# adrianalbert/domain-transfer-GAN

Hardware: AMD Instinct MI355X
Metric: training images/sec, 256x256 Augmented CycleGAN step, 1/2/4/8 MI355X (higher is better)
Workload: dtype f32 tensors; conv products as 3 bf16 MFMAs on hi/lo-split fp32 operands (~2^-17 operand rounding), fp32 accumulate; parity vs the reference goldens: losses / single-pass images / cycle reconstructions <= 1e-3 on every fixture at step 0 (measured rec_A / rec_B <= 7.9e-4, profiles/r06_rec_errors.txt)

## Files before the change

### domain-transfer-gan_amd/csrc/conv_patch.hip

```cpp
#include "common.h"
#include "conv_internal.h"

typedef __bf16 bf16x8 __attribute__((ext_vector_type(8)));
typedef float f32x4 __attribute__((ext_vector_type(4)));
typedef unsigned u32x4 __attribute__((ext_vector_type(4)));

namespace {
constexpr int PT_TH = 8, PT_TW = 16;
constexpr int PT_PIX = 320;
constexpr int PT_PLANE = PT_PIX * 8;
constexpr int PT_IMG = 4 * PT_PLANE;
}

template <bool REFLECT>
__global__ __launch_bounds__(256) void conv_patch16_x3(const float *__restrict__ in, const __bf16 *__restrict__ wp,
                                                       const float *__restrict__ bias, float *__restrict__ out, Geom g,
                                                       Taps taps, int dymin, int dxmin, int PH, int PW, unsigned in_bytes,
                                                       long long w_lo_elems)
{
    __shared__ __attribute__((aligned(16))) __bf16 Ap[2 * PT_IMG];
    const int tid = threadIdx.x, lane = tid & 63, wave = __builtin_amdgcn_readfirstlane(tid >> 6);
    const int tiles_x = (g.GW + PT_TW - 1) / PT_TW, tiles_y = (g.GH + PT_TH - 1) / PT_TH;
    const int nwg_ = gridDim.x, bid_ = blockIdx.x, xq_ = nwg_ >> 3, xr_ = nwg_ & 7, xcd_ = bid_ & 7;
    int b = (xcd_ < xr_ ? xcd_ * (xq_ + 1) : xr_ * (xq_ + 1) + (xcd_ - xr_) * xq_) + (bid_ >> 3);
    const int tx = b % tiles_x; b /= tiles_x;
    const int ty = b % tiles_y;
    const int n = b / tiles_y;
    const int gy0 = ty * PT_TH, gx0 = tx * PT_TW;

    const __amdgpu_buffer_rsrc_t rin = __builtin_amdgcn_make_buffer_rsrc((void *)in, 0, in_bytes, 0x00020000);
    const int npp = PH * PW;
    constexpr int NIT = 4 * PT_PIX / 256;
    static_assert(4 * PT_PIX % 256 == 0, "patch items per thread");
    f32x4 plo[NIT], phi[NIT];
#pragma unroll
    for (int it = 0; it < NIT; ++it) {
        const int i = tid + 256 * it;
        const int u = i / PT_PIX, pp = i - u * PT_PIX;
        const int py = pp / PW, px = pp - py * PW;
        int iy = gy0 + py + dymin, ix = gx0 + px + dxmin;
        bool ok = pp < npp;
        if (REFLECT) {
            ok = ok && iy > -g.Hin && iy < 2 * g.Hin - 1 && ix > -g.Win && ix < 2 * g.Win - 1;
            iy = iy < 0 ? -iy : iy;
            iy = iy >= g.Hin ? 2 * (g.Hin - 1) - iy : iy;
            ix = ix < 0 ? -ix : ix;
            ix = ix >= g.Win ? 2 * (g.Win - 1) - ix : ix;
        } else {
            ok = ok && (unsigned)iy < (unsigned)g.Hin && (unsigned)ix < (unsigned)g.Win;
        }
        const unsigned off = (unsigned)(((n * g.Hin + iy) * g.Win + ix) * g.Cin + 8 * u) * 4u;
        plo[it] = __builtin_bit_cast(f32x4, __builtin_amdgcn_raw_buffer_load_b128(rin, acg_masked_off(off, ok), 0, 0));
        phi[it] = __builtin_bit_cast(f32x4, __builtin_amdgcn_raw_buffer_load_b128(rin, acg_masked_off(off + 16u, ok), 0, 0));
    }
#pragma unroll
    for (int it = 0; it < NIT; ++it) {
        const int i = tid + 256 * it;
        const int u = i / PT_PIX, pp = i - u * PT_PIX;
        if (pp >= npp) continue;
        const float v[8] = {plo[it][0], plo[it][1], plo[it][2], plo[it][3], phi[it][0], phi[it][1], phi[it][2], phi[it][3]};
        acg_u32x4 hi, lo;
        acg_split8(v, hi, lo);
        *(acg_u32x4 *)&Ap[u * PT_PLANE + pp * 8] = hi;
        *(acg_u32x4 *)&Ap[PT_IMG + u * PT_PLANE + pp * 8] = lo;
    }
    __syncthreads();

    const int pl = lane >> 4, lr = lane & 15;
    f32x4 acc[2] = {{0.f, 0.f, 0.f, 0.f}, {0.f, 0.f, 0.f, 0.f}};
    const long long boff = ((long long)(pl >> 1) * g.ncols_pad + lr) * 16 + (pl & 1) * 8;
    const long long tap_stride = (long long)(g.Cin / 16) * g.ncols_pad * 16;
    constexpr int PF = 7;
    const int tap_v = taps.pk[lane < taps.n ? lane : 0];
    bf16x8 bh[PF], bl[PF];
    auto bload = [&](int t, bf16x8 &h, bf16x8 &l) {
        const int tw = __builtin_amdgcn_readlane(tap_v, t < taps.n ? t : 0) >> 16;
        const __bf16 *wt = wp + tw * tap_stride + boff;
        h = *(const bf16x8 *)wt;
        l = *(const bf16x8 *)(wt + w_lo_elems);
    };
    auto tap_mma = [&](int t, const bf16x8 &ch, const bf16x8 &cl) {
        const int pk = __builtin_amdgcn_readlane(tap_v, t);
        const int dy = ((pk << 24) >> 24) - dymin, dx = ((pk << 16) >> 24) - dxmin;
#pragma unroll
        for (int r = 0; r < 2; ++r) {
            const int pp = (wave * 2 + r + dy) * PW + dx + lr;
            const bf16x8 ah = *(const bf16x8 *)&Ap[pl * PT_PLANE + pp * 8];
            const bf16x8 al = *(const bf16x8 *)&Ap[PT_IMG + pl * PT_PLANE + pp * 8];
            acc[r] = __builtin_amdgcn_mfma_f32_16x16x32_bf16(al, ch, acc[r], 0, 0, 0);
            acc[r] = __builtin_amdgcn_mfma_f32_16x16x32_bf16(ah, cl, acc[r], 0, 0, 0);
            acc[r] = __builtin_amdgcn_mfma_f32_16x16x32_bf16(ah, ch, acc[r], 0, 0, 0);
        }
    };
    const int nfull = taps.n / PF * PF;
    if (nfull > 0) {
#pragma unroll
        for (int j = 0; j < PF; ++j) bload(j, bh[j], bl[j]);
    }
    for (int t0 = 0; t0 < nfull; t0 += PF) {
#pragma unroll
        for (int j = 0; j < PF; ++j) {
            tap_mma(t0 + j, bh[j], bl[j]);
            bload(t0 + j + PF, bh[j], bl[j]);
        }
    }
    for (int t = nfull; t < taps.n; ++t) {
        bf16x8 ch, cl;
        bload(t, ch, cl);
        tap_mma(t, ch, cl);
    }

    const float bv = (bias != nullptr && lr < g.Cout) ? bias[lr] : 0.f;
#pragma unroll
    for (int r = 0; r < 2; ++r) {
        const int gy = gy0 + wave * 2 + r;
#pragma unroll
        for (int k = 0; k < 4; ++k) {
            const int gx = gx0 + 4 * pl + k;
            if (gy < g.GH && gx < g.GW && lr < g.Cout)
                out[(((long long)n * g.Hout + gy) * g.Wout + gx) * g.Cout + lr] = acg_apply_act_ch(acc[r][k] + bv, g.act, lr);
        }
    }
}

template <bool REFLECT>
__global__ __launch_bounds__(256) __attribute__((amdgpu_waves_per_eu(4, 4))) void conv_patchn_x3(const float *__restrict__ in, const __bf16 *__restrict__ wn,
                                                      const float *__restrict__ bias, float *__restrict__ out, Geom g,
                                                      int dymin, int dxmin, int KH, int KW, unsigned in_bytes)
{
    __shared__ __attribute__((aligned(16))) __bf16 Ap[2 * PT_IMG];
    const int tid = threadIdx.x, lane = tid & 63, wave = __builtin_amdgcn_readfirstlane(tid >> 6);
    const int tiles_x = (g.GW + PT_TW - 1) / PT_TW, tiles_y = (g.GH + PT_TH - 1) / PT_TH;
    const int nwg_ = gridDim.x, bid_ = blockIdx.x, xq_ = nwg_ >> 3, xr_ = nwg_ & 7, xcd_ = bid_ & 7;
    int b = (xcd_ < xr_ ? xcd_ * (xq_ + 1) : xr_ * (xq_ + 1) + (xcd_ - xr_) * xq_) + (bid_ >> 3);
    const int tx = b % tiles_x; b /= tiles_x;
    const int ty = b % tiles_y;
    const int n = b / tiles_y;
    const int gy0 = ty * PT_TH, gx0 = tx * PT_TW;
    const int PH = PT_TH + KH - 1, PW = PT_TW + KW - 1;

    const __amdgpu_buffer_rsrc_t rin = __builtin_amdgcn_make_buffer_rsrc((void *)in, 0, in_bytes, 0x00020000);
    const int npp = PH * PW;
    constexpr int NIT = 4 * PT_PIX / 256;
    f32x4 plo[NIT], phi[NIT];
#pragma unroll
    for (int it = 0; it < NIT; ++it) {
        const int i = tid + 256 * it;
        const int u = i / PT_PIX, pp = i - u * PT_PIX;
        const int py = pp / PW, px = pp - py * PW;
        int iy = gy0 + py + dymin, ix = gx0 + px + dxmin;
        bool ok = pp < npp;
        if (REFLECT) {
            ok = ok && iy > -g.Hin && iy < 2 * g.Hin - 1 && ix > -g.Win && ix < 2 * g.Win - 1;
            iy = iy < 0 ? -iy : iy;
            iy = iy >= g.Hin ? 2 * (g.Hin - 1) - iy : iy;
            ix = ix < 0 ? -ix : ix;
            ix = ix >= g.Win ? 2 * (g.Win - 1) - ix : ix;
        } else {
            ok = ok && (unsigned)iy < (unsigned)g.Hin && (unsigned)ix < (unsigned)g.Win;
        }
        const unsigned off = (unsigned)(((n * g.Hin + iy) * g.Win + ix) * g.Cin + 8 * u) * 4u;
        plo[it] = __builtin_bit_cast(f32x4, __builtin_amdgcn_raw_buffer_load_b128(rin, acg_masked_off(off, ok), 0, 0));
        phi[it] = __builtin_bit_cast(f32x4, __builtin_amdgcn_raw_buffer_load_b128(rin, acg_masked_off(off + 16u, ok), 0, 0));
    }
    const int KU = KW + 3, S = KH * KU;
    constexpr int NSW = (7 * 10 + 3) / 4, PF = 6;
    bf16x8 bh[PF], bl[PF];
    auto bload = [&](int k, bf16x8 &h, bf16x8 &l) {
        int s = wave + 4 * k;
        s = s < S ? s : S - 1;
        h = *(const bf16x8 *)(wn + (long long)s * 512 + lane * 8);
        l = *(const bf16x8 *)(wn + (long long)(S + s) * 512 + lane * 8);
    };
#pragma unroll
    for (int k = 0; k < PF; ++k) bload(k, bh[k], bl[k]);
#pragma unroll
    for (int it = 0; it < NIT; ++it) {
        const int i = tid + 256 * it;
        const int u = i / PT_PIX, pp = i - u * PT_PIX;
        if (pp >= npp) continue;
        const float v[8] = {plo[it][0], plo[it][1], plo[it][2], plo[it][3], phi[it][0], phi[it][1], phi[it][2], phi[it][3]};
        acg_u32x4 hi, lo;
        acg_split8(v, hi, lo);
        *(acg_u32x4 *)&Ap[u * PT_PLANE + pp * 8] = hi;
        *(acg_u32x4 *)&Ap[PT_IMG + u * PT_PLANE + pp * 8] = lo;
    }
    __syncthreads();

    const int kg = lane >> 4, m = lane & 15, br = m >> 2, bc = m & 3;
    f32x4 acc[2] = {{0.f, 0.f, 0.f, 0.f}, {0.f, 0.f, 0.f, 0.f}};
    const int a0 = kg * PT_PLANE + (br * PW + 4 * bc) * 8;
#pragma unroll
    for (int k = 0; k < NSW; ++k) {
        const int s = wave + 4 * k;
        if (s < S) {
            const int ry = s / KU, u = s - ry * KU;
#pragma unroll
            for (int mt = 0; mt < 2; ++mt) {
                const int e = a0 + ((4 * mt + ry) * PW + u) * 8;
                const bf16x8 ah = *(const bf16x8 *)&Ap[e];
                const bf16x8 al = *(const bf16x8 *)&Ap[PT_IMG + e];
                acc[mt] = __builtin_amdgcn_mfma_f32_16x16x32_bf16(al, bh[k % PF], acc[mt], 0, 0, 0);
                acc[mt] = __builtin_amdgcn_mfma_f32_16x16x32_bf16(ah, bl[k % PF], acc[mt], 0, 0, 0);
                acc[mt] = __builtin_amdgcn_mfma_f32_16x16x32_bf16(ah, bh[k % PF], acc[mt], 0, 0, 0);
            }
        }
        if (k + PF < NSW) bload(k + PF, bh[k % PF], bl[k % PF]);
    }
    __syncthreads();
    float *red = (float *)Ap;
#pragma unroll
    for (int mt = 0; mt < 2; ++mt)
#pragma unroll
        for (int r = 0; r < 4; ++r) red[((wave * 2 + mt) * 4 + r) * 64 + lane] = acc[mt][r];
    __syncthreads();
    if (wave < 2) {
        const int mt = wave, c = lane & 3, dxo = (lane >> 2) & 3, q = lane >> 4;
        const float bv = (bias != nullptr && c < g.Cout) ? bias[c] : 0.f;
        const int gy = gy0 + 4 * mt + q;
#pragma unroll
        for (int r = 0; r < 4; ++r) {
            float v = red[((0 * 2 + mt) * 4 + r) * 64 + lane];
#pragma unroll
            for (int w = 1; w < 4; ++w) v += red[((w * 2 + mt) * 4 + r) * 64 + lane];
            const int gx = gx0 + 4 * r + dxo;
            if (gy < g.GH && gx < g.GW)
                out[(((long long)n * g.Hout + gy) * g.Wout + gx) * 4 + c] = acg_apply_act_ch(v + bv, g.act, c);
        }
    }
}

static bool patchn_window(const Taps &t, int *ymin, int *xmin, int *KH, int *KW)
{
    int y0 = t.dy[0], y1 = t.dy[0], x0 = t.dx[0], x1 = t.dx[0];
    for (int i = 1; i < t.n; ++i) {
        y0 = t.dy[i] < y0 ? t.dy[i] : y0; y1 = t.dy[i] > y1 ? t.dy[i] : y1;
        x0 = t.dx[i] < x0 ? t.dx[i] : x0; x1 = t.dx[i] > x1 ? t.dx[i] : x1;
    }
    const int kh = y1 - y0 + 1, kw = x1 - x0 + 1;
    if (kh != kw || kh * kw != t.n || kh < 2 || kh > 7) return false;
    unsigned long long seen = 0;
    bool all_fwd = true, all_bwd = true;
    for (int i = 0; i < t.n; ++i) {
        const int pos = (t.dy[i] - y0) * kw + (t.dx[i] - x0);
        if (seen >> pos & 1ull) return false;
        seen |= 1ull << pos;
        const int skh = t.w[i] / kw, skw = t.w[i] - skh * kw;
        all_fwd = all_fwd && skh == t.dy[i] - y0 && skw == t.dx[i] - x0;
        all_bwd = all_bwd && skh == kh - 1 - (t.dy[i] - y0) && skw == kw - 1 - (t.dx[i] - x0);
    }
    if (!all_fwd && !all_bwd) return false;
    *ymin = y0; *xmin = x0; *KH = kh; *KW = kw;
    return true;
}

bool acg_conv_patchn_ok(const Geom &g, const Taps &t)
{
    if (g_acg_precision != ACG_PREC_BF16X3 || g_acg_conv_impl != ACG_IMPL_MFMA || g.thin || g.fold_p || g.stats) return false;
    if (g.Cin != 32 || g.Cout != 4 || g.os != 1 || g.is != 1 || g.oy0 != 0 || g.ox0 != 0 || t.n < 4) return false;
    int a, b, kh, kw;
    if (!patchn_window(t, &a, &b, &kh, &kw)) return false;
    return (PT_TH + kh - 1) * (PT_TW + kw - 1) <= PT_PIX && g.Hin >= 2 && g.Win >= 2;
}

int acg_conv_patchn_launch(const float *in, const void *wn, const float *bias, float *out, const Geom &g, const Taps &t, hipStream_t st)
{
    int ymin, xmin, KH, KW;
    ACG_REQUIRE(acg_conv_patchn_ok(g, t) && patchn_window(t, &ymin, &xmin, &KH, &KW), "conv_patchn_x3: unsupported geometry");
    const long long nimg = g.Mtot / ((long long)g.GH * g.GW);
    const long long in_bytes = nimg * g.Hin * g.Win * g.Cin * 4;
    ACG_REQUIRE(in_bytes < (1LL << 32), "conv_patchn_x3: gathered tensor exceeds the 4 GiB buffer-addressing limit");
    const long long blocks = nimg * ((g.GH + PT_TH - 1) / PT_TH) * ((g.GW + PT_TW - 1) / PT_TW);
    if (g.reflect)
        hipLaunchKernelGGL((conv_patchn_x3<true>), dim3((unsigned)blocks), dim3(256), 0, st, in, (const __bf16 *)wn, bias, out, g, ymin, xmin, KH, KW, (unsigned)in_bytes);
    else
        hipLaunchKernelGGL((conv_patchn_x3<false>), dim3((unsigned)blocks), dim3(256), 0, st, in, (const __bf16 *)wn, bias, out, g, ymin, xmin, KH, KW, (unsigned)in_bytes);
    ACG_CHECK_LAUNCH("conv_patchn_x3");
    acg_note_kernel("conv_patchn_x3<REFLECT=%d> (%dx%d window, %d K steps)", g.reflect ? 1 : 0, KH, KW, KH * (KW + 3));
    return ACG_OK;
}

namespace {
constexpr int TR_PW = PT_TW + 8;
constexpr int TR_PHMAX = PT_TH + 6;
constexpr int TR_PLANE = TR_PHMAX * TR_PW * 4;
}
template <bool REFLECT>
__global__ __launch_bounds__(256) void conv_thinrow_x3(const float *__restrict__ in, const __bf16 *__restrict__ wr,
                                                       const float *__restrict__ bias, float *__restrict__ out, Geom g,
                                                       int dymin, int dxmin, int KH, unsigned in_bytes)
{
    __shared__ __attribute__((aligned(16))) float smem[PT_TH * PT_TW * 32 + 512];
    static_assert(sizeof(smem) >= 2 * TR_PLANE * sizeof(__bf16), "patch fits the tile buffer");
    __bf16 *const Ap = (__bf16 *)smem;
    const int tid = threadIdx.x, lane = tid & 63, wave = __builtin_amdgcn_readfirstlane(tid >> 6);
    const int tiles_x = (g.GW + PT_TW - 1) / PT_TW, tiles_y = (g.GH + PT_TH - 1) / PT_TH;
    const int nwg_ = gridDim.x, bid_ = blockIdx.x, xq_ = nwg_ >> 3, xr_ = nwg_ & 7, xcd_ = bid_ & 7;
    int b = (xcd_ < xr_ ? xcd_ * (xq_ + 1) : xr_ * (xq_ + 1) + (xcd_ - xr_) * xq_) + (bid_ >> 3);
    const int tx = b % tiles_x; b /= tiles_x;
    const int ty = b % tiles_y;
    const int n = b / tiles_y;
    const int gy0 = ty * PT_TH, gx0 = tx * PT_TW;
    const int PH = PT_TH + KH - 1;

    constexpr int PF = 3;
    const int kg = lane >> 4, lr = lane & 15;
    bf16x8 bh[PF][2], bl[PF][2];
    auto bload = [&](int ry, bf16x8 (&h)[2], bf16x8 (&l)[2]) {
        const int r = ry < KH ? ry : KH - 1;
#pragma unroll
        for (int ct = 0; ct < 2; ++ct) {
            const long long e = ((long long)(r * 4 + kg) * 32 + ct * 16 + lr) * 8;
            h[ct] = *(const bf16x8 *)(wr + e);
            l[ct] = *(const bf16x8 *)(wr + (long long)KH * 1024 + e);
        }
    };
#pragma unroll
    for (int k = 0; k < PF; ++k) bload(k, bh[k], bl[k]);

    const __amdgpu_buffer_rsrc_t rin = __builtin_amdgcn_make_buffer_rsrc((void *)in, 0, in_bytes, 0x00020000);
    constexpr int NIT = (TR_PHMAX * TR_PW + 255) / 256;
    f32x4 pv[NIT];
#pragma unroll
    for (int it = 0; it < NIT; ++it) {
        const int pp = tid + 256 * it;
        const int py = pp / TR_PW, px = pp - py * TR_PW;
        int iy = gy0 + py + dymin, ix = gx0 + px + dxmin;
        bool ok = py < PH;
        if (REFLECT) {
            ok = ok && iy > -g.Hin && iy < 2 * g.Hin - 1 && ix > -g.Win && ix < 2 * g.Win - 1;
            iy = iy < 0 ? -iy : iy;
            iy = iy >= g.Hin ? 2 * (g.Hin - 1) - iy : iy;
            ix = ix < 0 ? -ix : ix;
            ix = ix >= g.Win ? 2 * (g.Win - 1) - ix : ix;
        } else {
            ok = ok && (unsigned)iy < (unsigned)g.Hin && (unsigned)ix < (unsigned)g.Win;
        }
        const unsigned off = (unsigned)(((n * g.Hin + iy) * g.Win + ix) * 4) * 4u;
        pv[it] = __builtin_bit_cast(f32x4, __builtin_amdgcn_raw_buffer_load_b128(rin, acg_masked_off(off, ok), 0, 0));
    }
#pragma unroll
    for (int it = 0; it < NIT; ++it) {
        const int pp = tid + 256 * it;
        if (pp >= PH * TR_PW) continue;
        typedef __bf16 bf16x2_t __attribute__((ext_vector_type(2)));
        typedef float f32x2_t __attribute__((ext_vector_type(2)));
        uint2 hi, lo;
        unsigned *hp = &hi.x, *lp = &lo.x;
#pragma unroll
        for (int q = 0; q < 2; ++q) {
            const unsigned h = __builtin_bit_cast(unsigned, __builtin_convertvector((f32x2_t){pv[it][2 * q], pv[it][2 * q + 1]}, bf16x2_t));
            const float ha = __builtin_bit_cast(float, h << 16), hb = __builtin_bit_cast(float, h & 0xffff0000u);
            hp[q] = h;
            lp[q] = __builtin_bit_cast(unsigned, __builtin_convertvector((f32x2_t){pv[it][2 * q] - ha, pv[it][2 * q + 1] - hb}, bf16x2_t));
        }
        *(uint2 *)&Ap[pp * 4] = hi;
        *(uint2 *)&Ap[TR_PLANE + pp * 4] = lo;
    }
    __syncthreads();

    f32x4 nsx[PT_TH * PT_TW * 8 / 256];
    if (g.ns_part != nullptr) {
#pragma unroll
        for (int k = 0; k < PT_TH * PT_TW * 8 / 256; ++k) {
            const int idx = tid + 256 * k, pix = idx >> 3, c4 = idx & 7;
            nsx[k] = *(const f32x4 *)(g.ns_x + (((long long)n * g.Hout + gy0 + pix / PT_TW) * g.Wout + gx0 + pix % PT_TW) * g.Cout + c4 * 4);
        }
    }
    f32x4 acc[2][2];
#pragma unroll
    for (int r = 0; r < 2; ++r)
#pragma unroll
        for (int ct = 0; ct < 2; ++ct) acc[r][ct] = (f32x4){0.f, 0.f, 0.f, 0.f};
    typedef unsigned u32x2 __attribute__((ext_vector_type(2)));
    auto afrag = [&](int e) {
        const u32x2 a = *(const u32x2 *)&Ap[e], c = *(const u32x2 *)&Ap[e + 4];
        return __builtin_bit_cast(bf16x8, (u32x4){a[0], a[1], c[0], c[1]});
    };
    const int a0 = ((wave * 2) * TR_PW + lr + 2 * kg) * 4;
#pragma unroll
    for (int ry = 0; ry < 7; ++ry) {
        if (ry < KH) {
#pragma unroll
            for (int r = 0; r < 2; ++r) {
                const int e = a0 + (r + ry) * TR_PW * 4;
                const bf16x8 ah = afrag(e), al = afrag(TR_PLANE + e);
#pragma unroll
                for (int ct = 0; ct < 2; ++ct) {
                    acc[r][ct] = __builtin_amdgcn_mfma_f32_16x16x32_bf16(al, bh[ry % PF][ct], acc[r][ct], 0, 0, 0);
                    acc[r][ct] = __builtin_amdgcn_mfma_f32_16x16x32_bf16(ah, bl[ry % PF][ct], acc[r][ct], 0, 0, 0);
                    acc[r][ct] = __builtin_amdgcn_mfma_f32_16x16x32_bf16(ah, bh[ry % PF][ct], acc[r][ct], 0, 0, 0);
                }
            }
        }
        if (ry + PF < 7) bload(ry + PF, bh[ry % PF], bl[ry % PF]);
    }

    __syncthreads();
    float *const tile = smem, *const red = smem + PT_TH * PT_TW * 32;
#pragma unroll
    for (int ct = 0; ct < 2; ++ct) {
        const int co = ct * 16 + lr;
        const float bv = (bias != nullptr && co < g.Cout) ? bias[co] : 0.f;
#pragma unroll
        for (int r = 0; r < 2; ++r)
#pragma unroll
            for (int k = 0; k < 4; ++k)
                tile[((wave * 2 + r) * PT_TW + 4 * kg + k) * 32 + co] = acg_apply_act(acc[r][ct][k] + bv, g.stats != nullptr ? (int)ACG_ACT_NONE : g.act);
    }
    __syncthreads();
    const bool nsum = g.ns_part != nullptr;
    const int nc4 = tid & 7;
    f32x4 ns1 = {0.f, 0.f, 0.f, 0.f}, ns2 = ns1, nmu = ns1, nrs = ns1, nga = {1.f, 1.f, 1.f, 1.f}, nbe = nga;
    const bool ns_relu = nsum && g.ns_act == ACG_ACT_RELU;
    if (nsum) {
        nmu = *(const f32x4 *)(g.ns_mean + n * 32 + nc4 * 4);
        nrs = *(const f32x4 *)(g.ns_rstd + n * 32 + nc4 * 4);
        if (ns_relu) {
            nga = *(const f32x4 *)(g.ns_gamma + g.ns_gstride * n + nc4 * 4);
            nbe = *(const f32x4 *)(g.ns_beta + g.ns_gstride * n + nc4 * 4);
        }
    }
#pragma unroll
    for (int k = 0; k < PT_TH * PT_TW * 8 / 256; ++k) {
        const int idx = tid + 256 * k, pix = idx >> 3, c4 = idx & 7;
        const int gy = gy0 + pix / PT_TW, gx = gx0 + pix % PT_TW;
        if (gy < g.GH && gx < g.GW && c4 * 4 < g.Cout) {
            const long long o = (((long long)n * g.Hout + gy) * g.Wout + gx) * g.Cout + c4 * 4;
            const f32x4 v = *(const f32x4 *)&tile[pix * 32 + c4 * 4];
            *(f32x4 *)(out + o) = v;
            if (nsum) {
                const f32x4 xh = (nsx[k] - nmu) * nrs;
#pragma unroll
                for (int q = 0; q < 4; ++q) {
                    const float gyv = (ns_relu && !(xh[q] * nga[q] + nbe[q] > 0.f)) ? 0.f : v[q];
                    ns1[q] += gyv;
                    ns2[q] += gyv * xh[q];
                }
            }
        }
    }
    if (nsum) {
        __syncthreads();
        *(f32x4 *)&tile[(tid >> 3) * 64 + nc4 * 8] = ns1;
        *(f32x4 *)&tile[(tid >> 3) * 64 + nc4 * 8 + 4] = ns2;
        __syncthreads();
        if (tid < 64) {
            const int c = tid & 31, which = tid >> 5;
            float a = 0.f;
#pragma unroll
            for (int r = 0; r < 32; ++r) a += tile[r * 64 + (c >> 2) * 8 + which * 4 + (c & 3)];
            g.ns_part[((long long)(n * tiles_y * tiles_x + ty * tiles_x + tx) * 2 + which) * 32 + c] = a;
        }
        return;
    }
    if (g.stats != nullptr) {
        const int c = tid & 31, h = tid >> 5;
        float sum = 0.f;
#pragma unroll
        for (int r = 0; r < 16; ++r) sum += tile[(h * 16 + r) * 32 + c];
        red[h * 32 + c] = sum;
        __syncthreads();
        float tot = 0.f;
#pragma unroll
        for (int q = 0; q < 8; ++q) tot += red[q * 32 + c];
        const float mu = tot * (1.f / (PT_TH * PT_TW));
        float sq = 0.f;
#pragma unroll
        for (int r = 0; r < 16; ++r) {
            const float dlt = tile[(h * 16 + r) * 32 + c] - mu;
            sq += dlt * dlt;
        }
        __syncthreads();
        red[h * 32 + c] = sq;
        __syncthreads();
        if (h == 0 && c < g.Cout) {
            float m2 = 0.f;
#pragma unroll
            for (int q = 0; q < 8; ++q) m2 += red[q * 32 + c];
            float *o = g.stats + ((long long)(n * g.stats_cpi + g.stats_chunk0 + ty * tiles_x + tx) * 2) * g.Cout + c;
            o[0] = mu;
            o[g.Cout] = m2;
        }
    }
}

bool acg_conv_thinrow_ok(const Geom &g, const Taps &t)
{
    if (g_acg_precision != ACG_PREC_BF16X3 || g_acg_conv_impl != ACG_IMPL_MFMA || !g.thin || g.fold_p || acg_act_kind(g.act) == ACG_ACT_SIGMOID) return false;
    if (g.Cin != 4 || g.Cout != 32 || g.ncols_pad != 32 || g.os != 1 || g.is != 1 || g.oy0 != 0 || g.ox0 != 0 || t.n < 4) return false;
    if (g.stats != nullptr && (g.GH % PT_TH != 0 || g.GW % PT_TW != 0 || g.act != ACG_ACT_NONE)) return false;
    if (g.ns_part != nullptr && (g.stats != nullptr || g.GH % PT_TH != 0 || g.GW % PT_TW != 0 || g.act != ACG_ACT_NONE || g.ns_x == nullptr ||
                                 g.ns_mean == nullptr || g.ns_rstd == nullptr || g.ns_mask != nullptr ||
                                 (g.ns_act != ACG_ACT_NONE && (g.ns_act != ACG_ACT_RELU || g.ns_gamma == nullptr || g.ns_beta == nullptr)) ||
                                 (g.ns_gstride != 0 && (g.ns_gstride < 32 || g.ns_gstride % 4 != 0))))
        return false;
    int a, b, kh, kw;
    return patchn_window(t, &a, &b, &kh, &kw) && g.Hin >= 2 && g.Win >= 2;
}

int acg_conv_thinrow_launch(const float *in, const void *wr, const float *bias, float *out, const Geom &g, const Taps &t, hipStream_t st)
{
    int ymin, xmin, KH, KW;
    ACG_REQUIRE(acg_conv_thinrow_ok(g, t) && patchn_window(t, &ymin, &xmin, &KH, &KW), "conv_thinrow_x3: unsupported geometry");
    ACG_REQUIRE(g.ns_part == nullptr || bias == nullptr, "conv_thinrow_x3: the norm sums ride on a plain data gradient (no bias)");
    const long long nimg = g.Mtot / ((long long)g.GH * g.GW);
    const long long in_bytes = nimg * g.Hin * g.Win * g.Cin * 4;
    ACG_REQUIRE(in_bytes < (1LL << 32), "conv_thinrow_x3: gathered tensor exceeds the 4 GiB buffer-addressing limit");
    const long long blocks = nimg * ((g.GH + PT_TH - 1) / PT_TH) * ((g.GW + PT_TW - 1) / PT_TW);
    if (g.reflect)
        hipLaunchKernelGGL((conv_thinrow_x3<true>), dim3((unsigned)blocks), dim3(256), 0, st, in, (const __bf16 *)wr, bias, out, g, ymin, xmin, KH, (unsigned)in_bytes);
    else
        hipLaunchKernelGGL((conv_thinrow_x3<false>), dim3((unsigned)blocks), dim3(256), 0, st, in, (const __bf16 *)wr, bias, out, g, ymin, xmin, KH, (unsigned)in_bytes);
    ACG_CHECK_LAUNCH("conv_thinrow_x3");
    acg_note_kernel("conv_thinrow_x3<REFLECT=%d%s> (%dx%d window)", g.reflect ? 1 : 0, g.ns_part != nullptr ? ",SUMS=1" : "", KH, KW);
    return ACG_OK;
}

bool acg_conv_patch16_ok(const Geom &g, const Taps &t)
{
    if (g_acg_precision != ACG_PREC_BF16X3 || g_acg_conv_impl != ACG_IMPL_MFMA || g.thin || g.fold_p) return false;
    if (g.Cin != 32 || (g.Cout != 16 && g.Cout != 4) || g.os != 1 || g.is != 1 || g.oy0 != 0 || g.ox0 != 0 || t.n < 1) return false;
    int ymin = t.dy[0], ymax = t.dy[0], xmin = t.dx[0], xmax = t.dx[0];
    for (int i = 1; i < t.n; ++i) {
        ymin = t.dy[i] < ymin ? t.dy[i] : ymin; ymax = t.dy[i] > ymax ? t.dy[i] : ymax;
        xmin = t.dx[i] < xmin ? t.dx[i] : xmin; xmax = t.dx[i] > xmax ? t.dx[i] : xmax;
    }
    return (PT_TH + ymax - ymin) * (PT_TW + xmax - xmin) <= PT_PIX && g.Hin >= 2 && g.Win >= 2;
}

int acg_conv_patch16_launch(const float *in, const void *wp, const float *bias, float *out, const Geom &g, const Taps &t0,
                            long long n_w_elems, hipStream_t st)
{
    const Taps t = acg_taps_pack(t0);
    int ymin = t.dy[0], ymax = t.dy[0], xmin = t.dx[0], xmax = t.dx[0];
    for (int i = 1; i < t.n; ++i) {
        ymin = t.dy[i] < ymin ? t.dy[i] : ymin; ymax = t.dy[i] > ymax ? t.dy[i] : ymax;
        xmin = t.dx[i] < xmin ? t.dx[i] : xmin; xmax = t.dx[i] > xmax ? t.dx[i] : xmax;
    }
    const int PH = PT_TH + ymax - ymin, PW = PT_TW + xmax - xmin;
    const long long nimg = g.Mtot / ((long long)g.GH * g.GW);
    const long long in_bytes = nimg * g.Hin * g.Win * g.Cin * 4;
    ACG_REQUIRE(in_bytes < (1LL << 32), "conv_patch16_x3: gathered tensor exceeds the 4 GiB buffer-addressing limit");
    const long long blocks = nimg * ((g.GH + PT_TH - 1) / PT_TH) * ((g.GW + PT_TW - 1) / PT_TW);
    if (g.reflect)
        hipLaunchKernelGGL((conv_patch16_x3<true>), dim3((unsigned)blocks), dim3(256), 0, st, in, (const __bf16 *)wp, bias, out, g, t,
                           ymin, xmin, PH, PW, (unsigned)in_bytes, n_w_elems);
    else
        hipLaunchKernelGGL((conv_patch16_x3<false>), dim3((unsigned)blocks), dim3(256), 0, st, in, (const __bf16 *)wp, bias, out, g, t,
                           ymin, xmin, PH, PW, (unsigned)in_bytes, n_w_elems);
    ACG_CHECK_LAUNCH("conv_patch16_x3");
    acg_note_kernel("conv_patch16_x3<REFLECT=%d>", g.reflect ? 1 : 0);
    return ACG_OK;
}
```

Baseline: 230.4.

## Make conv_patchn_x3 persistent with double-buffered patch prefetch

Turns the Cin=32→Cout=4 patch conv into a persistent kernel on a fixed grid of 512 workgroups that walk tiles in XCD-aware order. The next tile's global patch load is issued before the current tile's MFMA loop, and its hi/lo split into a second LDS buffer overlaps the reduction. All weight fragments now stay resident in registers, and the row divide is replaced with a reciprocal multiply. The cost is double the LDS and lower occupancy (waves_per_eu 2), which may limit latency hiding. This is one kernel within a full training step.

After: 230.1. Within noise of the previous version (-0.2%).

```diff
diff --git a/domain-transfer-gan_amd/csrc/conv_patch.hip b/domain-transfer-gan_amd/csrc/conv_patch.hip
--- a/domain-transfer-gan_amd/csrc/conv_patch.hip
+++ b/domain-transfer-gan_amd/csrc/conv_patch.hip
@@ -10,6 +10,8 @@
 constexpr int PT_PIX = 320;
 constexpr int PT_PLANE = PT_PIX * 8;
 constexpr int PT_IMG = 4 * PT_PLANE;
+constexpr int PATCHN_GRID = 512;
+static_assert(PATCHN_GRID % 8 == 0, "tile order of conv_patchn_x3");
 }
 
 template <bool REFLECT>
@@ -124,109 +126,135 @@
 }
 
 template <bool REFLECT>
-__global__ __launch_bounds__(256) __attribute__((amdgpu_waves_per_eu(4, 4))) void conv_patchn_x3(const float *__restrict__ in, const __bf16 *__restrict__ wn,
+__global__ __launch_bounds__(256) __attribute__((amdgpu_waves_per_eu(2, 2))) void conv_patchn_x3(const float *__restrict__ in, const __bf16 *__restrict__ wn,
                                                       const float *__restrict__ bias, float *__restrict__ out, Geom g,
-                                                      int dymin, int dxmin, int KH, int KW, unsigned in_bytes)
-{
-    __shared__ __attribute__((aligned(16))) __bf16 Ap[2 * PT_IMG];
+                                                      int dymin, int dxmin, int KH, int KW, unsigned in_bytes, int ntiles)
+{
+    __shared__ __attribute__((aligned(16))) __bf16 Ap[2 * 2 * PT_IMG];
     const int tid = threadIdx.x, lane = tid & 63, wave = __builtin_amdgcn_readfirstlane(tid >> 6);
     const int tiles_x = (g.GW + PT_TW - 1) / PT_TW, tiles_y = (g.GH + PT_TH - 1) / PT_TH;
-    const int nwg_ = gridDim.x, bid_ = blockIdx.x, xq_ = nwg_ >> 3, xr_ = nwg_ & 7, xcd_ = bid_ & 7;
-    int b = (xcd_ < xr_ ? xcd_ * (xq_ + 1) : xr_ * (xq_ + 1) + (xcd_ - xr_) * xq_) + (bid_ >> 3);
-    const int tx = b % tiles_x; b /= tiles_x;
-    const int ty = b % tiles_y;
-    const int n = b / tiles_y;
-    const int gy0 = ty * PT_TH, gx0 = tx * PT_TW;
-    const int PH = PT_TH + KH - 1, PW = PT_TW + KW - 1;
+    const int PH = PT_TH + KH - 1, PW = PT_TW + KW - 1, npp = PH * PW;
+    const int xq_ = ntiles >> 3, xr_ = ntiles & 7;
+    auto tile_of = [&](int v, int &n, int &gy0, int &gx0) {
+        const int xcd_ = v & 7;
+        int b = (xcd_ < xr_ ? xcd_ * (xq_ + 1) : xr_ * (xq_ + 1) + (xcd_ - xr_) * xq_) + (v >> 3);
+        const int tx = b % tiles_x; b /= tiles_x;
+        const int ty = b % tiles_y;
+        n = b / tiles_y;
+        gy0 = ty * PT_TH; gx0 = tx * PT_TW;
+    };
 
     const __amdgpu_buffer_rsrc_t rin = __builtin_amdgcn_make_buffer_rsrc((void *)in, 0, in_bytes, 0x00020000);
-    const int npp = PH * PW;
     constexpr int NIT = 4 * PT_PIX / 256;
+    const int rpw = 65536 / PW + 1;
     f32x4 plo[NIT], phi[NIT];
-#pragma unroll
-    for (int it = 0; it < NIT; ++it) {
-        const int i = tid + 256 * it;
-        const int u = i / PT_PIX, pp = i - u * PT_PIX;
-        const int py = pp / PW, px = pp - py * PW;
-        int iy = gy0 + py + dymin, ix = gx0 + px + dxmin;
-        bool ok = pp < npp;
-        if (REFLECT) {
-            ok = ok && iy > -g.Hin && iy < 2 * g.Hin - 1 && ix > -g.Win && ix < 2 * g.Win - 1;
-            iy = iy < 0 ? -iy : iy;
-            iy = iy >= g.Hin ? 2 * (g.Hin - 1) - iy : iy;
-            ix = ix < 0 ? -ix : ix;
-            ix = ix >= g.Win ? 2 * (g.Win - 1) - ix : ix;
-        } else {
-            ok = ok && (unsigned)iy < (unsigned)g.Hin && (unsigned)ix < (unsigned)g.Win;
-        }
-        const unsigned off = (unsigned)(((n * g.Hin + iy) * g.Win + ix) * g.Cin + 8 * u) * 4u;
-        plo[it] = __builtin_bit_cast(f32x4, __builtin_amdgcn_raw_buffer_load_b128(rin, acg_masked_off(off, ok), 0, 0));
-        phi[it] = __builtin_bit_cast(f32x4, __builtin_amdgcn_raw_buffer_load_b128(rin, acg_masked_off(off + 16u, ok), 0, 0));
-    }
+    auto tid_now = [&]() { int t = tid; asm volatile("" : "+v"(t)); return t; };
+    auto pload = [&](int n, int gy0, int gx0) {
+        const int tl = tid_now();
+#pragma unroll
+        for (int it = 0; it < NIT; ++it) {
+            const int i = tl + 256 * it;
+            const int u = i / PT_PIX, pp = i - u * PT_PIX;
+            const int py = pp * rpw >> 16, px = pp - py * PW;
+            int iy = gy0 + py + dymin, ix = gx0 + px + dxmin;
+            bool ok = pp < npp;
+            if (REFLECT) {
+                ok = ok && iy > -g.Hin && iy < 2 * g.Hin - 1 && ix > -g.Win && ix < 2 * g.Win - 1;
+                iy = iy < 0 ? -iy : iy;
+                iy = iy >= g.Hin ? 2 * (g.Hin - 1) - iy : iy;
+                ix = ix < 0 ? -ix : ix;
+                ix = ix >= g.Win ? 2 * (g.Win - 1) - ix : ix;
+            } else {
+                ok = ok && (unsigned)iy < (unsigned)g.Hin && (unsigned)ix < (unsigned)g.Win;
+            }
+            const unsigned off = (unsigned)(((n * g.Hin + iy) * g.Win + ix) * g.Cin + 8 * u) * 4u;
+            plo[it] = __builtin_bit_cast(f32x4, __builtin_amdgcn_raw_buffer_load_b128(rin, acg_masked_off(off, ok), 0, 0));
+            phi[it] = __builtin_bit_cast(f32x4, __builtin_amdgcn_raw_buffer_load_b128(rin, acg_masked_off(off + 16u, ok), 0, 0));
+        }
+    };
+    auto psplit = [&](__bf16 *buf) {
+        const int tl = tid_now();
+#pragma unroll
+        for (int it = 0; it < NIT; ++it) {
+            const int i = tl + 256 * it;
+            const int u = i / PT_PIX, pp = i - u * PT_PIX;
+            if (pp >= npp) continue;
+            const float v[8] = {plo[it][0], plo[it][1], plo[it][2], plo[it][3], phi[it][0], phi[it][1], phi[it][2], phi[it][3]};
+            acg_u32x4 hi, lo;
+            acg_split8(v, hi, lo);
+            *(acg_u32x4 *)&buf[u * PT_PLANE + pp * 8] = hi;
+            *(acg_u32x4 *)&buf[PT_IMG + u * PT_PLANE + pp * 8] = lo;
+        }
+    };
+    int v = blockIdx.x, n, gy0, gx0;
+    tile_of(v, n, gy0, gx0);
+    pload(n, gy0, gx0);
     const int KU = KW + 3, S = KH * KU;
-    constexpr int NSW = (7 * 10 + 3) / 4, PF = 6;
-    bf16x8 bh[PF], bl[PF];
-    auto bload = [&](int k, bf16x8 &h, bf16x8 &l) {
+    constexpr int NSW = (7 * 10 + 3) / 4;
+    bf16x8 bh[NSW], bl[NSW];
+#pragma unroll
+    for (int k = 0; k < NSW; ++k) {
         int s = wave + 4 * k;
         s = s < S ? s : S - 1;
-        h = *(const bf16x8 *)(wn + (long long)s * 512 + lane * 8);
-        l = *(const bf16x8 *)(wn + (long long)(S + s) * 512 + lane * 8);
-    };
-#pragma unroll
-    for (int k = 0; k < PF; ++k) bload(k, bh[k], bl[k]);
-#pragma unroll
-    for (int it = 0; it < NIT; ++it) {
-        const int i = tid + 256 * it;
-        const int u = i / PT_PIX, pp = i - u * PT_PIX;
-        if (pp >= npp) continue;
-        const float v[8] = {plo[it][0], plo[it][1], plo[it][2], plo[it][3], phi[it][0], phi[it][1], phi[it][2], phi[it][3]};
-        acg_u32x4 hi, lo;
-        acg_split8(v, hi, lo);
-        *(acg_u32x4 *)&Ap[u * PT_PLANE + pp * 8] = hi;
-        *(acg_u32x4 *)&Ap[PT_IMG + u * PT_PLANE + pp * 8] = lo;
-    }
+        bh[k] = *(const bf16x8 *)(wn + (long long)s * 512 + lane * 8);
+        bl[k] = *(const bf16x8 *)(wn + (long long)(S + s) * 512 + lane * 8);
+    }
+    psplit(Ap);
     __syncthreads();
 
     const int kg = lane >> 4, m = lane & 15, br = m >> 2, bc = m & 3;
-    f32x4 acc[2] = {{0.f, 0.f, 0.f, 0.f}, {0.f, 0.f, 0.f, 0.f}};
     const int a0 = kg * PT_PLANE + (br * PW + 4 * bc) * 8;
-#pragma unroll
-    for (int k = 0; k < NSW; ++k) {
-        const int s = wave + 4 * k;
-        if (s < S) {
-            const int ry = s / KU, u = s - ry * KU;
-#pragma unroll
-            for (int mt = 0; mt < 2; ++mt) {
-                const int e = a0 + ((4 * mt + ry) * PW + u) * 8;
-                const bf16x8 ah = *(const bf16x8 *)&Ap[e];
-                const bf16x8 al = *(const bf16x8 *)&Ap[PT_IMG + e];
-                acc[mt] = __builtin_amdgcn_mfma_f32_16x16x32_bf16(al, bh[k % PF], acc[mt], 0, 0, 0);
-                acc[mt] = __builtin_amdgcn_mfma_f32_16x16x32_bf16(ah, bl[k % PF], acc[mt], 0, 0, 0);
-                acc[mt] = __builtin_amdgcn_mfma_f32_16x16x32_bf16(ah, bh[k % PF], acc[mt], 0, 0, 0);
+    const float bv = (bias != nullptr && (lane & 3) < g.Cout) ? bias[lane & 3] : 0.f;
+    for (int cur = 0;; cur ^= 1) {
+        __bf16 *const Ac = Ap + cur * (2 * PT_IMG), *const An = Ap + (cur ^ 1) * (2 * PT_IMG);
+        const int vn = v + gridDim.x;
+        const bool more = vn < ntiles;
+        int nn = 0, ngy0 = 0, ngx0 = 0;
+        if (more) {
+            tile_of(vn, nn, ngy0, ngx0);
+            pload(nn, ngy0, ngx0);
+        }
+        f32x4 acc[2] = {{0.f, 0.f, 0.f, 0.f}, {0.f, 0.f, 0.f, 0.f}};
+        int ry = 0, u = wave;
+        asm volatile("" : "+s"(u));
+#pragma unroll
+        for (int k = 0; k < NSW; ++k, u += 4) {
+            if (u >= KU) { u -= KU; ++ry; }
+            if (ry < KH) {
+#pragma unroll
+                for (int mt = 0; mt < 2; ++mt) {
+                    const int e = a0 + ((4 * mt + ry) * PW + u) * 8;
+                    const bf16x8 ah = *(const bf16x8 *)&Ac[e];
+                    const bf16x8 al = *(const bf16x8 *)&Ac[PT_IMG + e];
+                    acc[mt] = __builtin_amdgcn_mfma_f32_16x16x32_bf16(al, bh[k], acc[mt], 0, 0, 0);
+                    acc[mt] = __builtin_amdgcn_mfma_f32_16x16x32_bf16(ah, bl[k], acc[mt], 0, 0, 0);
+                    acc[mt] = __builtin_amdgcn_mfma_f32_16x16x32_bf16(ah, bh[k], acc[mt], 0, 0, 0);
+                }
             }
         }
-        if (k + PF < NSW) bload(k + PF, bh[k % PF], bl[k % PF]);
-    }
-    __syncthreads();
-    float *red = (float *)Ap;
-#pragma unroll
-    for (int mt = 0; mt < 2; ++mt)
-#pragma unroll
-        for (int r = 0; r < 4; ++r) red[((wave * 2 + mt) * 4 + r) * 64 + lane] = acc[mt][r];
-    __syncthreads();
-    if (wave < 2) {
-        const int mt = wave, c = lane & 3, dxo = (lane >> 2) & 3, q = lane >> 4;
-        const float bv = (bias != nullptr && c < g.Cout) ? bias[c] : 0.f;
-        const int gy = gy0 + 4 * mt + q;
-#pragma unroll
-        for (int r = 0; r < 4; ++r) {
-            float v = red[((0 * 2 + mt) * 4 + r) * 64 + lane];
-#pragma unroll
-            for (int w = 1; w < 4; ++w) v += red[((w * 2 + mt) * 4 + r) * 64 + lane];
-            const int gx = gx0 + 4 * r + dxo;
-            if (gy < g.GH && gx < g.GW)
-                out[(((long long)n * g.Hout + gy) * g.Wout + gx) * 4 + c] = acg_apply_act_ch(v + bv, g.act, c);
-        }
+        __syncthreads();
+        if (more) psplit(An);
+        float *red = (float *)Ac;
+#pragma unroll
+        for (int mt = 0; mt < 2; ++mt)
+#pragma unroll
+            for (int r = 0; r < 4; ++r) red[((wave * 2 + mt) * 4 + r) * 64 + lane] = acc[mt][r];
+        __syncthreads();
+        if (wave < 2) {
+            const int mt = wave, c = lane & 3, dxo = (lane >> 2) & 3, q = lane >> 4;
+            const int gy = gy0 + 4 * mt + q;
+#pragma unroll
+            for (int r = 0; r < 4; ++r) {
+                float t = red[((0 * 2 + mt) * 4 + r) * 64 + lane];
+#pragma unroll
+                for (int w = 1; w < 4; ++w) t += red[((w * 2 + mt) * 4 + r) * 64 + lane];
+                const int gx = gx0 + 4 * r + dxo;
+                if (gy < g.GH && gx < g.GW)
+                    out[(((long long)n * g.Hout + gy) * g.Wout + gx) * 4 + c] = acg_apply_act_ch(t + bv, g.act, c);
+            }
+        }
+        if (!more) break;
+        v = vn; n = nn; gy0 = ngy0; gx0 = ngx0;
     }
 }
 
@@ -270,13 +298,15 @@
     const long long nimg = g.Mtot / ((long long)g.GH * g.GW);
     const long long in_bytes = nimg * g.Hin * g.Win * g.Cin * 4;
     ACG_REQUIRE(in_bytes < (1LL << 32), "conv_patchn_x3: gathered tensor exceeds the 4 GiB buffer-addressing limit");
-    const long long blocks = nimg * ((g.GH + PT_TH - 1) / PT_TH) * ((g.GW + PT_TW - 1) / PT_TW);
+    const long long tiles = nimg * ((g.GH + PT_TH - 1) / PT_TH) * ((g.GW + PT_TW - 1) / PT_TW);
+    ACG_REQUIRE(tiles < (1LL << 31), "conv_patchn_x3: tile count");
+    const int blocks = tiles < PATCHN_GRID ? (int)tiles : PATCHN_GRID;
     if (g.reflect)
-        hipLaunchKernelGGL((conv_patchn_x3<true>), dim3((unsigned)blocks), dim3(256), 0, st, in, (const __bf16 *)wn, bias, out, g, ymin, xmin, KH, KW, (unsigned)in_bytes);
+        hipLaunchKernelGGL((conv_patchn_x3<true>), dim3((unsigned)blocks), dim3(256), 0, st, in, (const __bf16 *)wn, bias, out, g, ymin, xmin, KH, KW, (unsigned)in_bytes, (int)tiles);
     else
-        hipLaunchKernelGGL((conv_patchn_x3<false>), dim3((unsigned)blocks), dim3(256), 0, st, in, (const __bf16 *)wn, bias, out, g, ymin, xmin, KH, KW, (unsigned)in_bytes);
+        hipLaunchKernelGGL((conv_patchn_x3<false>), dim3((unsigned)blocks), dim3(256), 0, st, in, (const __bf16 *)wn, bias, out, g, ymin, xmin, KH, KW, (unsigned)in_bytes, (int)tiles);
     ACG_CHECK_LAUNCH("conv_patchn_x3");
-    acg_note_kernel("conv_patchn_x3<REFLECT=%d> (%dx%d window, %d K steps)", g.reflect ? 1 : 0, KH, KW, KH * (KW + 3));
+    acg_note_kernel("conv_patchn_x3<REFLECT=%d> (%dx%d window, %d K steps, %d workgroups walk %lld tiles)", g.reflect ? 1 : 0, KH, KW, KH * (KW + 3), blocks, tiles);
     return ACG_OK;
 }
 
```
